# Epiphany-f/PSL-SLAM

Hardware: AMD Instinct MI355X
Metric: frames/sec ORB+line extract+match, 640x480 RGB-D, 1/2/4/8 MI355X (higher is better)
Workload: dtype u8; 1 GPU; configs[2]: 640x480 synthetic structure scene at the configured line load ('sticks': non-overlapping high-contrast bars), ORB 1000/1.2/8 FAST 20/7 + LSD (LSD_REFINE_ADV) / merge / top-200 / LBD + LIL pairing + RGB-D line glue (isLineGood, crossings, planes) extract, SearchByProjection(cur,last) + LSDmatcher::match, frames resident in HBM; scene=sticks, distinct_frames_per_batch=256, streams=1, launcher=none, multi_gpu=single GPU, lsd_refine=LSD_REFINE_ADV, lbd_sample_bytes_per_frame=2654242

## Files before the change

include/pslfe.h:

```cpp
#ifndef PSLFE_H
#define PSLFE_H
#include <stddef.h>
#include <stdint.h>

#ifdef __cplusplus
extern "C" {
#endif

#define PSLFE_OK 0
#define PSLFE_E_INVALID (-1)
#define PSLFE_E_NODEVICE (-2)
#define PSLFE_E_HIP (-3)
#define PSLFE_E_CAPACITY (-4)
#define PSLFE_E_STATE (-5)

#define PSLFE_MAX_LEVELS 16
#define PSLFE_FAN_CAP 4096

typedef struct PslKeyPoint {
    float x, y;
    float size;
    float angle;
    float response;
    int32_t octave;
// ... 78 lines not shown
int pslfe_line_levels(const pslfe_line* line);
float pslfe_line_scale_factor(const pslfe_line* line);
int pslfe_line_scale_factors(const pslfe_line* line, float* scale, float* inv_scale, float* sigma2, float* inv_sigma2);

int pslfe_lsd_detect(pslfe_line* line, const uint8_t* gray, int w, int h, int stride, float* segments, int cap, int* n);
int pslfe_line_debug_gradient(pslfe_line* line, int frame, int* W, int* H, double* scaled, float* angle_deg, double* modgrad);
#define PSLFE_MATH_ATANF 0
#define PSLFE_MATH_TANF 1
#define PSLFE_MATH_SINCOSF 2
#define PSLFE_MATH_FAST_ATAN2 3
#define PSLFE_MATH_ATAN2F 4
#define PSLFE_MATH_FDIV 5
#define PSLFE_MATH_SQRTF 6
#define PSLFE_MATH_CVROUND_F 7
#define PSLFE_MATH_LOG 8
#define PSLFE_MATH_EXP 9
#define PSLFE_MATH_LOG10 10
#define PSLFE_MATH_POW_POS 11
#define PSLFE_MATH_SINH_SMALL 12
#define PSLFE_MATH_LOG_GAMMA 13
#define PSLFE_MATH_GLIBC_SIN 14
#define PSLFE_MATH_GLIBC_COS 15
#define PSLFE_MATH_COS_SIN_F64 16
#define PSLFE_MATH_COS_SIN_2PI_F32 17
#define PSLFE_MATH_RATIO_INV 18
#define PSLFE_MATH_DDIV 19
#define PSLFE_MATH_DSQRT 20
#define PSLFE_MATH_CVROUND_D 21
#define PSLFE_MATH_COUNT 22
int pslfe_debug_math(pslfe_ctx* ctx, int fn, size_t n, const void* a, const void* b, void* out0, void* out1);
#define PSLFE_NFA_FIRST (-2)
int pslfe_line_debug_nfa(pslfe_line* line, int w, int h, int phase, int nframes, const int32_t* nrect, int rect_cap,
                         const double* p_lognfa, const int32_t* nk, double* vals, double* tail, double* log_nt);

int pslfe_line_extract(pslfe_line* line, const uint8_t* gray, int w, int h, int stride, PslKeyLine* kls, uint8_t* desc,
                       double* lineEq, int cap, int* n);
int pslfe_line_extract_batch_device(pslfe_line* line, const uint8_t* d_gray, int nframes, int w, int h, int stride,
                                    size_t frame_stride);
int pslfe_line_results_device(pslfe_line* line, const PslKeyLine** d_kls, const uint8_t** d_desc, const double** d_lineEq,
                              const int32_t** d_counts, int* kl_cap);
int pslfe_line_fetch(pslfe_line* line, int frame, PslKeyLine* kls, uint8_t* desc, double* lineEq, int cap, int* n, int* status);
int pslfe_line_segments_fetch(pslfe_line* line, int frame, float* segments, int cap, int* n);

int pslfe_line_optimize_and_merge(pslfe_line* line, const float* segments, int nseg, int w, int h, PslKeyLine* kls, int cap, int* n);
int pslfe_lbd_compute(pslfe_line* line, const uint8_t* gray, int w, int h, int stride, const PslKeyLine* kls, int nkl,
                      uint8_t* desc, float* fdesc);
int pslfe_line_debug_sobel(pslfe_line* line, int frame, int16_t* dx, int16_t* dy);

int pslfe_lil_pair(pslfe_line* line, const float* lines, int nlines, float radius, float fanThr, int imgCols, int imgRows,
                   float* fans, int cap, int* nfans);
int pslfe_line_pair_batch_device(pslfe_line* line, float radius, float fanThr);
int pslfe_line_fans_fetch(pslfe_line* line, int frame, float* fans, int cap, int* nfans);
int pslfe_line_fans_device(pslfe_line* line, const float** d_fans, const int32_t** d_nfans, int* fan_stride);

int pslfe_line_match_batch_device(pslfe_line* line, int shift, float nnr, int32_t* d_matches12, int32_t* d_nmatches);

int pslfe_hamming_knn2(pslfe_ctx* ctx, const uint8_t* q, int nq, const uint8_t* t, int nt,
                       int32_t* idx, int32_t* dist);
int pslfe_hamming_knn2_device(pslfe_ctx* ctx, const uint8_t* d_q, int nq, const uint8_t* d_t, int nt,
                              int32_t* d_idx, int32_t* d_dist);

typedef struct PslProjQuery {
    float u, v;
    float radius;
    float ur;
    int32_t min_level;
// ... 559 lines not shown
```

psl-slam_amd/__init__.py:

```python
import ctypes as C
import os

import numpy as np

_HERE = os.path.dirname(os.path.abspath(__file__))
LIB_PATH = os.path.join(_HERE, "libpslfe.so")

KEYPOINT_DTYPE = np.dtype([("x", "<f4"), ("y", "<f4"), ("size", "<f4"), ("angle", "<f4"), ("response", "<f4"),
                           ("octave", "<i4"), ("class_id", "<i4")])
KEYLINE_DTYPE = np.dtype([("angle", "<f4"), ("class_id", "<i4"), ("octave", "<i4"), ("pt_x", "<f4"), ("pt_y", "<f4"),
                          ("response", "<f4"), ("size", "<f4"), ("startPointX", "<f4"), ("startPointY", "<f4"),
                          ("endPointX", "<f4"), ("endPointY", "<f4"), ("sPointInOctaveX", "<f4"),
                          ("sPointInOctaveY", "<f4"), ("ePointInOctaveX", "<f4"), ("ePointInOctaveY", "<f4"),
                          ("lineLength", "<f4"), ("numOfPixels", "<i4")])
PROJQUERY_DTYPE = np.dtype([("u", "<f4"), ("v", "<f4"), ("radius", "<f4"), ("ur", "<f4"), ("min_level", "<i4"),
                            ("max_level", "<i4"), ("angle", "<f4"), ("blocks", "<i4")])
BOWQUERY_DTYPE = np.dtype([("start", "<i4"), ("len", "<i4"), ("angle", "<f4")])
CAMERA_DTYPE = np.dtype([(k, "<f4") for k in ("fx", "fy", "cx", "cy", "k1", "k2", "p1", "p2", "k3", "bf")])
assert KEYPOINT_DTYPE.itemsize == 28 and KEYLINE_DTYPE.itemsize == 68 and PROJQUERY_DTYPE.itemsize == 32
POSE_DTYPE = np.dtype([("R", "<f4", (9,)), ("t", "<f4", (3,))])
LASTPOINT_DTYPE = np.dtype([("x", "<f4"), ("y", "<f4"), ("z", "<f4"), ("state", "<i4")])
MAPPOINT_DTYPE = np.dtype([(k, "<f4") for k in ("x", "y", "z", "nx", "ny", "nz", "min_dist", "max_dist")])
assert POSE_DTYPE.itemsize == 48 and LASTPOINT_DTYPE.itemsize == 16 and MAPPOINT_DTYPE.itemsize == 32
LASTPOINT_NONE, LASTPOINT_NO_OBS, LASTPOINT_OBS, LASTPOINT_OUTLIER = 0, 1, 2, 8
# ... 1250 lines not shown
    else:
        assert b is None, f"{fn} takes one argument"
    return MATH_FUNCTIONS.index(fn), a, b, np.zeros(len(a), t0), None if t1 is None else np.zeros(len(a), t1)


def debug_math(fn, a, b=None, ctx=None):
    ctx = ctx or default_context()
    i, a, b, o0, o1 = math_arrays(fn, a, b)
    _check(lib().pslfe_debug_math(ctx._h, C.c_int(i), C.c_size_t(len(a)), _ptr(a), _ptr(b), _ptr(o0), _ptr(o1)), "pslfe_debug_math")
    return o0 if o1 is None else (o0, o1)


NFA_FIRST = -2


def _line_debug_nfa(self, w, h, phase, nrect, p_lognfa, nk):
    nrect = np.ascontiguousarray(nrect, np.int32).ravel()
    F = len(nrect)
    pl = np.ascontiguousarray(p_lognfa, np.float64)
    nk = np.ascontiguousarray(nk, np.int32)
    R = pl.shape[1]
    assert pl.shape == (F, R, 2) and nk.shape == (F, R, 5, 2), (pl.shape, nk.shape)
    vals = np.full((F, R, 5), np.nan)
    tail = np.full((F, R, 5), np.nan)
    lognt = C.c_double()
    _check(lib().pslfe_line_debug_nfa(self._h, C.c_int(w), C.c_int(h), C.c_int(phase), C.c_int(F), _ptr(nrect), C.c_int(R), _ptr(pl), _ptr(nk),
                                      _ptr(vals), _ptr(tail), C.byref(lognt)), "pslfe_line_debug_nfa")
    return vals, tail, lognt.value


LINEextractor.debug_nfa = _line_debug_nfa


def _lsd_search_by_geom_appearance(self, kl_last, desc_last, kl_cur, desc_cur, has_mapline, desc_th, bounds):
    k1 = np.ascontiguousarray(kl_last, KEYLINE_DTYPE)
    k2 = np.ascontiguousarray(kl_cur, KEYLINE_DTYPE)
    d1 = np.ascontiguousarray(desc_last, np.uint8).reshape(-1, 32)
    d2 = np.ascontiguousarray(desc_cur, np.uint8).reshape(-1, 32)
    hm = np.ascontiguousarray(has_mapline, np.uint8)
    m12 = np.full(max(len(k1), 1), -1, np.int32)
    asg = np.full(max(len(k2), 1), -1, np.int32)
    n = C.c_int()
    _check(lib().pslfe_line_search_by_geom_appearance(self.ctx._h, _ptr(k1), _ptr(d1), C.c_int(len(k1)), _ptr(k2), _ptr(d2), C.c_int(len(k2)),
                                                      _ptr(hm), C.c_float(desc_th), *[C.c_float(b) for b in bounds], _ptr(m12), _ptr(asg),
                                                      C.byref(n)), "pslfe_line_search_by_geom_appearance")
    return n.value, m12[:len(k1)], asg[:len(k2)]


def _lsd_frame_bf_match(self, ldesc1, ldesc2, TH):
    d1 = np.ascontiguousarray(ldesc1, np.uint8).reshape(-1, 32)
    d2 = np.ascontiguousarray(ldesc2, np.uint8).reshape(-1, 32)
    lm = np.full(max(len(d1), 1), -1, np.int32)
    _check(lib().pslfe_line_frame_bf_match(self.ctx._h, _ptr(d1), C.c_int(len(d1)), _ptr(d2), C.c_int(len(d2)), C.c_float(self.mfNNratio),
                                           C.c_float(TH), _ptr(lm)), "pslfe_line_frame_bf_match")
    return lm[:len(d1)]


LSDmatcher.SearchByGeomNApearance = _lsd_search_by_geom_appearance
LSDmatcher.FrameBFMatch = _lsd_frame_bf_match


def associate_planes(planes, points, map_planes, dTh, aTh, live=True, map_bad=None, ctx=None):
    ctx = ctx or default_context()
    p = np.ascontiguousarray(planes, np.float32).reshape(-1, 4)
    q = np.ascontiguousarray(points, np.float64).reshape(-1, 15)
    m = np.ascontiguousarray(map_planes, np.float32).reshape(-1, 4)
# ... 748 lines not shown
```

psl-slam_amd/csrc/line_kernels3.h:

```cpp
#ifndef PSL_LINE_KERNELS3_H
#define PSL_LINE_KERNELS3_H

#include "line_kernels.h"
#include "psl_log_gamma.h"

struct LsdnRect { double x1, y1, x2, y2, width, theta, dx, dy, prec, p; };
struct LsdnGeom {
    int ya, yb;
    int lefty, righty;
    long long minx, fl, sl, fr, sr;
};

__device__ __forceinline__ void lsdn_cswap(long long& a, long long& b) { const long long lo = a < b ? a : b, hi = a < b ? b : a; a = lo; b = hi; }

__device__ __forceinline__ void lsdn_geom(const LsdnRect& r, int H, LsdnGeom* G) {
    const double half_width = r.width / 2.0;
    const double dyhw = PSL_DMUL(r.dy, half_width), dxhw = PSL_DMUL(r.dx, half_width);
    int cx[4] = {(int)PSL_DSUB(r.x1, dyhw), (int)PSL_DSUB(r.x2, dyhw), (int)PSL_DADD(r.x2, dyhw), (int)PSL_DADD(r.x1, dyhw)};
    int cy[4] = {(int)PSL_DADD(r.y1, dxhw), (int)PSL_DADD(r.y2, dxhw), (int)PSL_DSUB(r.y2, dxhw), (int)PSL_DSUB(r.y1, dxhw)};
    long long k[4];
#pragma unroll
    for (int i = 0; i < 4; ++i) k[i] = (long long)cx[i] * 4294967296ll + ((long long)cy[i] + 2147483648ll);
    lsdn_cswap(k[0], k[1]); lsdn_cswap(k[2], k[3]); lsdn_cswap(k[0], k[2]); lsdn_cswap(k[1], k[3]); lsdn_cswap(k[1], k[2]);
#pragma unroll
// ... 33 lines not shown
    G->yb = mxy >= H ? H - 1 : mxy;
}

__device__ __forceinline__ void lsdn_row_span(const LsdnGeom& G, int y, int W, int* xa, int* xb) {
    const int n = y - G.ya;
    int c1 = (y < G.lefty ? y : G.lefty) - G.ya; c1 = c1 < 0 ? 0 : c1;
    int d1 = (y < G.righty ? y : G.righty) - G.ya; d1 = d1 < 0 ? 0 : d1;
    const long long L = G.minx + G.fl * c1 + G.sl * (n - c1);
    const long long R = G.minx + G.fr * d1 + G.sr * (n - d1);
    *xa = (int)(L < 0 ? 0 : (L > W ? W : L));
    *xb = (int)(R >= W ? W - 1 : (R < -1 ? -1 : R));
}

#ifndef PSL_NFA_BYROW_MIN
#define PSL_NFA_BYROW_MIN 4
#endif
#ifndef PSL_NFA_BYROW_T
#define PSL_NFA_BYROW_T 3
#endif
template <int GL>
__device__ __forceinline__ int lsdn_group_sum(int v) {
#pragma unroll
    for (int o = GL / 2; o > 0; o >>= 1) v += __shfl_xor(v, o);
    return v;
}

template <int GL>
__device__ __forceinline__ int lsdn_group_max(int v) {
#pragma unroll
    for (int o = GL / 2; o > 0; o >>= 1) { const int u = __shfl_xor(v, o); v = u > v ? u : v; }
    return v;
}

template <int NP, int GL>
__device__ __forceinline__ void lsdn_count(const float* __restrict__ ang, int W, const LsdnGeom& G, double theta, const double* prec, int lane, int* total, int* alg) {
    int al[NP];
#pragma unroll
    for (int j = 0; j < NP; ++j) al[j] = 0;
    const float theta_deg = (float)(theta * 57.295779513082320877);
    float pdeg[NP];
#pragma unroll
    for (int j = 0; j < NP; ++j) pdeg[j] = (float)(prec[j] * 57.295779513082320877);
    auto pixel = [&](float a) {
        if (a == PSL_LSD_NOTDEF) return;
        float d = __builtin_fabsf(theta_deg - a);
        const float d2 = __builtin_fabsf(d - 360.0f);
        d = d > 270.0f ? d2 : d;
        bool close = __builtin_fabsf(d - 270.0f) < 2e-3f;
#pragma unroll
        for (int j = 0; j < NP; ++j) close = close || __builtin_fabsf(d - pdeg[j]) < 2e-3f;
        if (!close) {
#pragma unroll
            for (int j = 0; j < NP; ++j) al[j] += d <= pdeg[j] ? 1 : 0;
        } else {
            const double f = lsdg_fold(PSL_DMUL((double)a, PSL_DEG2RAD), theta);
#pragma unroll
            for (int j = 0; j < NP; ++j) al[j] += f <= prec[j] ? 1 : 0;
        }
    };
    const int nrows = G.yb - G.ya + 1;
    int tot = 0;
    if (nrows >= PSL_NFA_BYROW_MIN) {
        for (int y = G.ya + lane; y <= G.yb; y += GL) {
            int xa, xb;
            lsdn_row_span(G, y, W, &xa, &xb);
            const int c = xb - xa + 1;
            tot += c > 0 ? c : 0;
            const float* row = ang + y * W;
            for (int x = xa; x <= xb; x += 4) {
                float a[4];
#pragma unroll
                for (int u = 0; u < 4; ++u) a[u] = x + u <= xb ? row[x + u] : PSL_LSD_NOTDEF;
#pragma unroll
                for (int u = 0; u < 4; ++u) pixel(a[u]);
            }
        }
        *total = lsdn_group_sum<GL>(tot);
    } else {
        int wmax = 0;
        for (int y = G.ya + lane; y <= G.yb; y += GL) {
            int xa, xb;
            lsdn_row_span(G, y, W, &xa, &xb);
            const int c = xb - xa + 1;
            tot += c > 0 ? c : 0;
            wmax = c > wmax ? c : wmax;
        }
        *total = lsdn_group_sum<GL>(tot);
        wmax = lsdn_group_max<GL>(wmax);
        if (nrows > 0 && wmax > 0) {
            const int nslots = nrows * wmax, row_step = GL / wmax, dx_step = GL - row_step * wmax;
            int row = lane / wmax, dx = lane - row * wmax;
            for (int s = lane; s < nslots; s += 4 * GL) {
                float a[4];
#pragma unroll
                for (int u = 0; u < 4; ++u) {
                    a[u] = PSL_LSD_NOTDEF;
                    if (s + GL * u < nslots) {
                        int xa, xb;
                        const int y = G.ya + row;
                        lsdn_row_span(G, y, W, &xa, &xb);
                        if (dx <= xb - xa) a[u] = ang[y * W + xa + dx];
                    }
                    dx += dx_step; row += row_step;
                    if (dx >= wmax) { dx -= wmax; ++row; }
                }
#pragma unroll
                for (int u = 0; u < 4; ++u) pixel(a[u]);
            }
        }
    }
#pragma unroll
    for (int j = 0; j < NP; ++j) alg[j] = lsdn_group_sum<GL>(al[j]);
}

struct LsdnGeomI { int ya, yb, lefty, righty, minx, fl, sl, fr, sr; };
typedef __attribute__((address_space(3))) const int lds_cint;

__device__ __forceinline__ void lsdn_row_span_i(lds_cint* g, int y, int W, int* xa, int* xb) {
    const int ya = g[0], lefty = g[2], righty = g[3], minx = g[4];
    const int n = y - ya;
    int c1 = (y < lefty ? y : lefty) - ya; c1 = c1 < 0 ? 0 : c1;
    int d1 = (y < righty ? y : righty) - ya; d1 = d1 < 0 ? 0 : d1;
    const int L = minx + g[5] * c1 + g[6] * (n - c1);
    const int R = minx + g[7] * d1 + g[8] * (n - d1);
    *xa = L < 0 ? 0 : (L > W ? W : L);
    *xb = R >= W ? W - 1 : (R < -1 ? -1 : R);
}

template <int GL>
__device__ __forceinline__ void lsdn_count_trials(const float* __restrict__ ang, int W, lds_cint* geo, double theta, double prec, int lane, int* total, int* alg) {
    const float theta_deg = (float)(theta * 57.295779513082320877), pdeg = (float)(prec * 57.295779513082320877);
    auto aligned = [&](float a) -> bool {
        if (a == PSL_LSD_NOTDEF) return false;
        float d = __builtin_fabsf(theta_deg - a);
        const float d2 = __builtin_fabsf(d - 360.0f);
        d = d > 270.0f ? d2 : d;
        if (__builtin_fabsf(d - 270.0f) < 2e-3f || __builtin_fabsf(d - pdeg) < 2e-3f) return lsdg_fold(PSL_DMUL((double)a, PSL_DEG2RAD), theta) <= prec;
        return d <= pdeg;
    };
    int ya = 0, yb = -1;
    bool any = false;
#pragma unroll
    for (int t = 0; t < 5; ++t) {
        const int a = geo[9 * t], b = geo[9 * t + 1];
        if (b >= a) {
            ya = !any || a < ya ? a : ya;
            yb = !any || b > yb ? b : yb;
            any = true;
        }
    }
    int tot[5], al[5];
#pragma unroll
    for (int t = 0; t < 5; ++t) { tot[t] = 0; al[t] = 0; }
    const bool by_row = yb - ya + 1 >= PSL_NFA_BYROW_T;
    for (int y = by_row ? ya + lane : ya; y <= yb; y += by_row ? GL : 1) {
        int xa[5], xb[5], ua = 0x7fffffff, ub = -1;
#pragma unroll
        for (int t = 0; t < 5; ++t) {
            xa[t] = 1; xb[t] = 0;
            if (y >= geo[9 * t] && y <= geo[9 * t + 1]) lsdn_row_span_i(geo + 9 * t, y, W, &xa[t], &xb[t]);
            if (xb[t] >= xa[t]) {
                if (by_row || lane == 0) tot[t] += xb[t] - xa[t] + 1;
                ua = xa[t] < ua ? xa[t] : ua; ub = xb[t] > ub ? xb[t] : ub;
            }
        }
        if (ub < ua) continue;
        const float* row = ang + y * W;
        const int step = by_row ? 1 : GL;
        for (int x = by_row ? ua : ua + lane; x <= ub; x += 4 * step) {
            float a[4];
#pragma unroll
            for (int u = 0; u < 4; ++u) a[u] = x + step * u <= ub ? row[x + step * u] : PSL_LSD_NOTDEF;
#pragma unroll
            for (int u = 0; u < 4; ++u) {
                if (aligned(a[u])) {
#pragma unroll
                    for (int t = 0; t < 5; ++t) al[t] += (x + step * u >= xa[t] && x + step * u <= xb[t]) ? 1 : 0;
                }
            }
        }
    }
#pragma unroll
    for (int t = 0; t < 5; ++t) { total[t] = lsdn_group_sum<GL>(tot[t]); alg[t] = lsdn_group_sum<GL>(al[t]); }
}

__device__ __forceinline__ bool lsdn_double_equal0(double a) {
    if (a == 0.0) return true;
    const double aa = fabs(a);
    const double abs_max = aa < 2.2250738585072014e-308 ? 2.2250738585072014e-308 : aa;
    return (aa / abs_max) <= PSL_DMUL(100.0, 2.2204460492503131e-16);
}

#define PSL_NFA_NP 11
struct LsdnTables {
    const double* lg;
    const double* logs;
    int lg_n;
    double p0, log_nt;
    const double* inv;
};

__device__ __forceinline__ double lsdn_lg(const LsdnTables& T, int i) { return i < T.lg_n ? T.lg[i] : lsdn_log_gamma((double)i); }

__device__ __forceinline__ int lsdn_tail_test_fast(double term, double bin_tail, double mult_term, int q, double log_nt) {
    const unsigned long long bits = (unsigned long long)__double_as_longlong(bin_tail);
    const int e = (int)((bits >> 52) & 0x7ff) - 1023;
    if (e <= -1022 || e >= 1024 || q < 2) return -1;
    const double tb = 0.1 * bin_tail;
    {
        const double a0 = -(double)e * 0.30102999566398120 - log_nt, a1 = -(double)(e + 1) * 0.30102999566398120 - log_nt;
        const double f0 = fabs(a0), f1 = fabs(a1);
// ... 32 lines not shown
__device__ __forceinline__ void lsdn_load(const double* __restrict__ r, LsdnRect* rec) {
    rec->x1 = r[0]; rec->y1 = r[1]; rec->x2 = r[2]; rec->y2 = r[3]; rec->width = r[4]; rec->theta = r[5]; rec->dx = r[6]; rec->dy = r[7];
    rec->prec = r[8]; rec->p = r[9];
}

#ifndef PSL_NFA_GL
#define PSL_NFA_GL 16
#endif

#ifndef PSL_NFA_COUNT_WAVES
#define PSL_NFA_COUNT_WAVES 8
#endif
template <int PH>
__global__ __launch_bounds__(256, PSL_NFA_COUNT_WAVES) void k_lsd_nfa_count(LineParams P, const float* __restrict__ angdeg, double* __restrict__ rects,
                                                          const int* __restrict__ nrect, const uint16_t* __restrict__ ulist, const int* __restrict__ ucount,
                                                          int2* __restrict__ counts, int2* __restrict__ count0) {
    static_assert(PH == PSL_NFA_FIRST || (PH >= 0 && PH <= 3), "phase -1 is counted by the first test's pass");
    constexpr int GPB = 256 / PSL_NFA_GL;
    __shared__ int s_geo[GPB * 45];
    const int frame = blockIdx.y, lane = threadIdx.x & (PSL_NFA_GL - 1);
    const int cnt = PH == PSL_NFA_FIRST ? (nrect[frame] < P.maxseg ? nrect[frame] : P.maxseg) : ucount[frame];
    const uint16_t* ul = ulist + (size_t)frame * P.maxseg;
    const float* ang = angdeg + (size_t)frame * P.W * P.H;
    for (int item = (int)blockIdx.x * GPB + (int)(threadIdx.x / PSL_NFA_GL); item < cnt; item += (int)gridDim.x * GPB) {
        const int idx = PH == PSL_NFA_FIRST ? item : (int)ul[item];
        const size_t o = (size_t)frame * P.maxseg + idx;
        double* rs = rects + o * PSL_LSD_RECT_F64;
        LsdnRect rec;
        lsdn_load(rs, &rec);
        LsdnGeom G;
        int2* out = counts + o * 5;
        if (PH == PSL_NFA_FIRST) {
            if (lane == 0) { rs[8] = P.prec; rs[9] = P.p; }
            double pr[6], pp = P.p;
            pr[0] = P.prec;
#pragma unroll
            for (int t = 0; t < 5; ++t) { pp = pp / 2; pr[t + 1] = PSL_DMUL(pp, PSL_PI); }
            int tot, kk[6];
            lsdn_geom(rec, P.H, &G);
            lsdn_count<6, PSL_NFA_GL>(ang, P.W, G, rec.theta, pr, lane, &tot, kk);
            if (lane == 0) {
                count0[o] = make_int2(tot, kk[0]);
#pragma unroll
                for (int t = 0; t < 5; ++t) out[t] = make_int2(tot, kk[t + 1]);
            }
        } else if (PH == 3) {
            if (!(PSL_DSUB(rec.width, 0.5) >= 0.5)) {
                if (lane < 5) out[lane] = make_int2(-1, 0);
                continue;
            }
            double pr[5], pp = rec.p;
#pragma unroll
            for (int t = 0; t < 5; ++t) { pp = pp / 2; pr[t] = PSL_DMUL(pp, PSL_PI); }
            int tot, kk[5];
            lsdn_geom(rec, P.H, &G);
            lsdn_count<5, PSL_NFA_GL>(ang, P.W, G, rec.theta, pr, lane, &tot, kk);
            if (lane == 0) {
#pragma unroll
                for (int t = 0; t < 5; ++t) out[t] = make_int2(tot, kk[t]);
            }
        } else {
            int* geo = &s_geo[(threadIdx.x / PSL_NFA_GL) * 45];
            if (lane < 5) {
                LsdnRect r = rec;
                bool valid = true;
                for (int t = 0; t <= lane; ++t) {
                    if (!(PSL_DSUB(r.width, 0.5) >= 0.5)) { valid = false; break; }
                    lsdn_shrink(r, PH);
                }
                int* g = geo + 9 * lane;
                g[0] = 0; g[1] = -2;
                if (valid) {
                    lsdn_geom(r, P.H, &G);
                    g[1] = -1;
                    if (G.yb >= G.ya) {
                        g[0] = G.ya; g[1] = G.yb; g[2] = G.lefty; g[3] = G.righty; g[4] = (int)G.minx;
                        g[5] = (int)G.fl; g[6] = (int)G.sl; g[7] = (int)G.fr; g[8] = (int)G.sr;
                    }
                }
            }
            __builtin_amdgcn_wave_barrier();
            int nn[5], kk[5];
            lsdn_count_trials<PSL_NFA_GL>(ang, P.W, (lds_cint*)geo, rec.theta, rec.prec, lane, nn, kk);
            if (lane == 0) {
#pragma unroll
                for (int t = 0; t < 5; ++t) out[t] = geo[9 * t + 1] == -2 ? make_int2(-1, 0) : make_int2(nn[t], kk[t]);
            }
            __builtin_amdgcn_wave_barrier();
        }
// ... 289 lines not shown
```

psl-slam_amd/csrc/pslfe_line.hip:

```cpp
#include <math.h>
#include <stdlib.h>
#include <string.h>

#include <algorithm>
#include <mutex>
#include <vector>

#include "line_kernels2.h"
#include "line_kernels3.h"
#include "pslfe_internal.h"

#ifndef PSL_NFA_COUNT_WGS
#define PSL_NFA_COUNT_WGS 4
#endif
#define PSL_GROW_LDS_USED_MAX (144u * 1024u)
#ifndef PSL_GROW_HELPER_FRAMES
#define PSL_GROW_HELPER_FRAMES 64
#endif
constexpr unsigned PSL_LINE_PIECES = 2;
constexpr unsigned PSL_LINE_FIRST_NUM = 7, PSL_LINE_FIRST_DEN = 12;

#define PSL_GROW_LDS_DEVICES 64
static std::mutex g_grow_lds_mu;
static size_t g_grow_lds_attr[PSL_GROW_LDS_DEVICES];
// ... 65 lines not shown
    float* d_tmplines = nullptr;

    PslDeviceBuffers mem;

    void release() {
        mem.release();
        gw = gh = 0;
        last_nframes = 0;
    }

    int prepare(int w, int h) {
        if (w == gw && h == gh) return PSLFE_OK;
        PSL_REQUIRE(w >= 16 && h >= 16 && w <= 8192 && h <= 8192, PSLFE_E_INVALID, "line: image %dx%d out of range", w, h);
        LineParams Q;
        memset(&Q, 0, sizeof(Q));
        Q.w = w; Q.h = h;
        Q.W = (int)nearbyint(w * 0.8);
        Q.H = (int)nearbyint(h * 0.8);
        Q.maxseg = PSL_MERGE_NMAX;
        Q.maxkl = std::max(1024, nfeatures);
        Q.nfeatures = nfeatures;
        {
            const double sigma = 0.6 / 0.8;
            const int ksize = 1 + 2 * (int)ceil(sigma * sqrt(2 * 3.0 * log(10.0)));
            PSL_REQUIRE(ksize == 7, PSLFE_E_INVALID, "line: unexpected LSD kernel size %d", ksize);
            const double scale2X = -0.5 / (sigma * sigma);
            double sum = 0;
            for (int i = 0; i < 7; ++i) { const double x = i - 3.0; Q.gk[i] = exp(scale2X * x * x); sum += Q.gk[i]; }
            sum = 1. / sum;
            for (int i = 0; i < 7; ++i) Q.gk[i] *= sum;
        }
        Q.prec = PSL_PI * 22.5 / 180;
        Q.p = 22.5 / 180;
        Q.rho = 2.0 / sin(Q.prec);
        {
            double q = Q.rho * Q.rho;
            while (sqrt(nextafter(q, INFINITY)) <= Q.rho) q = nextafter(q, INFINITY);
            while (sqrt(q) > Q.rho) q = nextafter(q, 0.0);
            Q.rho_q = q;
        }
        const double LOG_NT = 5 * (log10((double)Q.W) + log10((double)Q.H)) / 2 + log10(11.0);
        Q.min_reg_size = (int)(size_t)(-LOG_NT / log10(Q.p));
        Q.log_nt = LOG_NT;
        Q.refine = refine;
        {
            float cf[5];
            double sum = 0;
            for (int i = 0; i < 5; ++i) { const double x = i - 2.0; cf[i] = (float)exp(-0.5 * x * x); sum += cf[i]; }
            sum = 1. / sum;
            for (int i = 0; i < 5; ++i) { cf[i] = (float)(cf[i] * sum); Q.lbdK[i] = (int)nearbyint((double)cf[i] * 256.0); }
        }
        {
            const int wb = 7, nb = 9;
            double u = (wb * 3 - 1) / 2, sigma = (wb * 2 + 1) / 2, inv = -1 / (2 * sigma * sigma);
            for (int i = 0; i < wb * 3; ++i) { const double d = i - u; Q.gaussL[i] = (float)exp(d * d * inv); }
            u = (nb * wb - 1) / 2; sigma = u; inv = -1 / (2 * sigma * sigma);
            for (int i = 0; i < nb * wb; ++i) { const double d = i - u; Q.gaussG[i] = (float)exp(d * d * inv); }
        }
        PSL_HIP(hipSetDevice(ctx->device));
        PSL_HIP(hipStreamSynchronize(ctx->stream));
        release();
        if (int rc = allocate(Q, w, h)) { release(); return rc; }
        P = Q;
        gw = w; gh = h;
        last_nframes = 0;
        return PSLFE_OK;
// ... 454 lines not shown
    }
#define PSL_NFA_DEBUG_EVAL(PH)                                                                                                                  \
    case PH:                                                                                                                                    \
        k_lsd_nfa_setup<PH><<<F, 256, 0, st>>>(P, line->NT, line->d_rects, line->d_nrect, d_ul, d_uc, line->d_counts, line->d_count0, line->d_vals, \
                                               line->d_sstate, line->d_stmp, line->d_slist, line->d_lcount);                                    \
        k_lsd_nfa_series<PH><<<dim3(PSL_NFA_NCLS, (F + PSL_NFA_FG - 1) / PSL_NFA_FG), 256, 0, st>>>(P, line->NT, (int)F, line->d_slist, line->d_lcount, \
                                                                                                    line->d_sstate);                            \
        break;
    switch (phase) {
        PSL_NFA_DEBUG_EVAL(PSL_NFA_FIRST)
        PSL_NFA_DEBUG_EVAL(-1)
        PSL_NFA_DEBUG_EVAL(0)
        PSL_NFA_DEBUG_EVAL(1)
        PSL_NFA_DEBUG_EVAL(2)
        PSL_NFA_DEBUG_EVAL(3)
    }
#undef PSL_NFA_DEBUG_EVAL
    PSL_HIP(hipGetLastError());
    std::vector<double> v(F * N * 5);
    std::vector<double2> ss(F * N * 5);
    PSL_HIP(hipMemcpyAsync(v.data(), line->d_vals, v.size() * sizeof(double), hipMemcpyDeviceToHost, st));
    PSL_HIP(hipMemcpyAsync(ss.data(), line->d_sstate, ss.size() * sizeof(double2), hipMemcpyDeviceToHost, st));
    PSL_HIP(hipStreamSynchronize(st));
    for (size_t f = 0; f < F; ++f)
        for (int r = 0; r < nrect[f]; ++r)
            for (int t = 0; t < TR; ++t) {
                vals[((size_t)f * rect_cap + r) * 5 + t] = v[(f * N + r) * 5 + t];
                tail[((size_t)f * rect_cap + r) * 5 + t] = ss[(f * N + r) * 5 + t].x;
            }
    if (log_nt) *log_nt = line->NT.log_nt;
    return PSLFE_OK;
}

int pslfe_line_extract_batch_device(pslfe_line* line, const uint8_t* d_gray, int nframes, int w, int h, int stride, size_t frame_stride) {
    PSL_REQUIRE(line && d_gray, PSLFE_E_INVALID, "pslfe_line_extract_batch_device: NULL argument");
    PSL_REQUIRE(nframes >= 1 && nframes <= line->max_batch, PSLFE_E_INVALID, "pslfe_line_extract_batch_device: nframes %d (max_batch %d)", nframes, line->max_batch);
    PSL_REQUIRE(stride >= w && (nframes == 1 || frame_stride >= (size_t)stride * h), PSLFE_E_INVALID, "pslfe_line_extract_batch_device: strides");
    return line->run_extract(d_gray, nframes, w, h, stride, frame_stride);
}

int pslfe_line_results_device(pslfe_line* line, const PslKeyLine** d_kls, const uint8_t** d_desc, const double** d_lineEq,
                              const int32_t** d_counts, int* kl_cap) {
    PSL_REQUIRE(line, PSLFE_E_INVALID, "pslfe_line_results_device: line is NULL");
    PSL_REQUIRE(line->last_nframes > 0, PSLFE_E_STATE, "pslfe_line_results_device: no batch extracted yet");
    if (d_kls) *d_kls = line->d_kls;
    if (d_desc) *d_desc = line->d_ldesc;
    if (d_lineEq) *d_lineEq = line->d_lineEq;
    if (d_counts) *d_counts = line->d_nkl;
    if (kl_cap) *kl_cap = line->P.maxkl;
    return PSLFE_OK;
}

int pslfe_line_fetch(pslfe_line* line, int frame, PslKeyLine* kls, uint8_t* desc, double* lineEq, int cap, int* n, int* status) {
    PSL_REQUIRE(line && n, PSLFE_E_INVALID, "pslfe_line_fetch: NULL argument");
    PSL_REQUIRE(line->last_nframes > 0 && frame >= 0 && frame < line->last_nframes, PSLFE_E_STATE, "pslfe_line_fetch: frame %d", frame);
    PSL_HIP(hipSetDevice(line->ctx->device));
    hipStream_t st = line->ctx->stream;
    int cnt = 0, stt = 0;
    PSL_HIP(hipMemcpyAsync(&cnt, line->d_nkl + frame, sizeof(int), hipMemcpyDeviceToHost, st));
    PSL_HIP(hipMemcpyAsync(&stt, line->d_status + frame, sizeof(int), hipMemcpyDeviceToHost, st));
    PSL_HIP(hipStreamSynchronize(st));
    *n = cnt;
    if (status) *status = stt;
    PSL_REQUIRE(cnt <= cap, PSLFE_E_CAPACITY, "pslfe_line_fetch: %d keylines, capacity %d", cnt, cap);
    if (cnt > 0) {
        const size_t o = (size_t)frame * line->P.maxkl;
// ... 179 lines not shown
```

Before: 36860 frames/s.

## Bin NFA alignment counts via exponent-bit histogram and bitmask popcounts

The LSD NFA count kernel used to compare each pixel's angle difference against every halved tolerance. Because those tolerances are successive powers of two, it now computes the bin straight from the float exponent bits and accumulates into a packed 64-bit histogram of 10-bit fields, flushed before any field can overflow. A double-precision fallback handles values near a bin edge. The refine counter builds a 32-bit aligned-pixel mask and uses popcount against span bitmasks in place of per-pixel comparisons over five ranges. A debug entry point and a startup check on the factor-of-two tolerance relation are also added.

```diff
diff --git a/include/pslfe.h b/include/pslfe.h
--- a/include/pslfe.h
+++ b/include/pslfe.h
@@ -134,6 +134,8 @@
 #define PSLFE_NFA_FIRST (-2)
 int pslfe_line_debug_nfa(pslfe_line* line, int w, int h, int phase, int nframes, const int32_t* nrect, int rect_cap,
                          const double* p_lognfa, const int32_t* nk, double* vals, double* tail, double* log_nt);
+int pslfe_line_debug_nfa_count(pslfe_line* line, int w, int h, int phase, int nframes, const int32_t* nrect, int rect_cap,
+                               const double* rects, const float* angle_deg, int32_t* nk, int32_t* first_nk);
 
 int pslfe_line_extract(pslfe_line* line, const uint8_t* gray, int w, int h, int stride, PslKeyLine* kls, uint8_t* desc,
                        double* lineEq, int cap, int* n);
diff --git a/psl-slam_amd/__init__.py b/psl-slam_amd/__init__.py
--- a/psl-slam_amd/__init__.py
+++ b/psl-slam_amd/__init__.py
@@ -1306,6 +1306,24 @@
 LINEextractor.debug_nfa = _line_debug_nfa
 
 
+def _line_debug_nfa_count(self, w, h, phase, nrect, rects, angle_deg):
+    nrect = np.ascontiguousarray(nrect, np.int32).ravel()
+    F = len(nrect)
+    rects = np.ascontiguousarray(rects, np.float64)
+    ang = np.ascontiguousarray(angle_deg, np.float32)
+    R = rects.shape[1]
+    W, H = int(round(w * 0.8)), int(round(h * 0.8))
+    assert rects.shape == (F, R, 12) and ang.shape == (F, H, W), (rects.shape, ang.shape, (F, H, W))
+    nk = np.full((F, R, 5, 2), -2, np.int32)
+    first = np.full((F, R, 2), -2, np.int32) if phase == NFA_FIRST else None
+    _check(lib().pslfe_line_debug_nfa_count(self._h, C.c_int(w), C.c_int(h), C.c_int(phase), C.c_int(F), _ptr(nrect), C.c_int(R), _ptr(rects),
+                                            _ptr(ang), _ptr(nk), _ptr(first) if first is not None else None), "pslfe_line_debug_nfa_count")
+    return nk, first
+
+
+LINEextractor.debug_nfa_count = _line_debug_nfa_count
+
+
 def _lsd_search_by_geom_appearance(self, kl_last, desc_last, kl_cur, desc_cur, has_mapline, desc_th, bounds):
     k1 = np.ascontiguousarray(kl_last, KEYLINE_DTYPE)
     k2 = np.ascontiguousarray(kl_cur, KEYLINE_DTYPE)
diff --git a/psl-slam_amd/csrc/line_kernels3.h b/psl-slam_amd/csrc/line_kernels3.h
--- a/psl-slam_amd/csrc/line_kernels3.h
+++ b/psl-slam_amd/csrc/line_kernels3.h
@@ -89,47 +89,67 @@
     return v;
 }
 
-template <int NP, int GL>
-__device__ __forceinline__ void lsdn_count(const float* __restrict__ ang, int W, const LsdnGeom& G, double theta, const double* prec, int lane, int* total, int* alg) {
-    int al[NP];
-#pragma unroll
-    for (int j = 0; j < NP; ++j) al[j] = 0;
+#define LSDN_FW 10
+#define LSDN_CAP ((1 << LSDN_FW) - 1)
+#define LSDN_SEG 1020
+static_assert(LSDN_SEG <= LSDN_CAP && LSDN_SEG % 4 == 0, "a piece of a row must fit in a histogram field");
+template <int NP, bool FIRST, int GL>
+__device__ __forceinline__ void lsdn_count(const float* __restrict__ ang, int W, const LsdnGeom& G, double theta, double prec0, double p, int lane, int* total, int* alg) {
+    static_assert(NP * LSDN_FW <= 64, "the histogram is one 64-bit register pair");
+    int cnt[NP];
+#pragma unroll
+    for (int f = 0; f < NP; ++f) cnt[f] = 0;
+    unsigned long long hist = 0;
+    auto flush = [&]() {
+#pragma unroll
+        for (int f = 0; f < NP; ++f) cnt[f] += (int)((hist >> (LSDN_FW * f)) & LSDN_CAP);
+        hist = 0;
+    };
     const float theta_deg = (float)(theta * 57.295779513082320877);
-    float pdeg[NP];
-#pragma unroll
-    for (int j = 0; j < NP; ++j) pdeg[j] = (float)(prec[j] * 57.295779513082320877);
+    constexpr int NH = FIRST ? NP - 1 : NP;
+    const double half = PSL_DMUL(p / 2, PSL_PI);
+    const float top = (float)((FIRST ? prec0 : half) * 57.295779513082320877);
+    const int topbits = __float_as_int(top);
+    const float margin = top >= 8e-3f * (float)(1 << NP) ? 2e-3f : __builtin_inff();
     auto pixel = [&](float a) {
         if (a == PSL_LSD_NOTDEF) return;
         float d = __builtin_fabsf(theta_deg - a);
         const float d2 = __builtin_fabsf(d - 360.0f);
         d = d > 270.0f ? d2 : d;
-        bool close = __builtin_fabsf(d - 270.0f) < 2e-3f;
-#pragma unroll
-        for (int j = 0; j < NP; ++j) close = close || __builtin_fabsf(d - pdeg[j]) < 2e-3f;
-        if (!close) {
-#pragma unroll
-            for (int j = 0; j < NP; ++j) al[j] += d <= pdeg[j] ? 1 : 0;
-        } else {
+        int c = ((topbits - __float_as_int(d)) >> 23) + 1;
+        c = c < 0 ? 0 : (c > NP ? NP : c);
+        const int lobits = topbits - (c << 23);
+        const float lo = __int_as_float(lobits), hi = __int_as_float(lobits + (1 << 23));
+        const float near = __builtin_fminf(__builtin_fminf(__builtin_fabsf(d - lo), __builtin_fabsf(d - hi)), __builtin_fabsf(d - 270.0f));
+        if (near < margin) {
             const double f = lsdg_fold(PSL_DMUL((double)a, PSL_DEG2RAD), theta);
-#pragma unroll
-            for (int j = 0; j < NP; ++j) al[j] += f <= prec[j] ? 1 : 0;
-        }
+            const long long e = ((__double_as_longlong(half) - __double_as_longlong(f)) >> 52) + 1;
+            c = e < 0 ? 0 : (e > NH ? NH : (int)e);
+            if (FIRST) c += f <= prec0 ? 1 : 0;
+        }
+        hist += 1ull << (LSDN_FW * NP - LSDN_FW * c);
     };
     const int nrows = G.yb - G.ya + 1;
     int tot = 0;
     if (nrows >= PSL_NFA_BYROW_MIN) {
+        int pend = 0;
         for (int y = G.ya + lane; y <= G.yb; y += GL) {
             int xa, xb;
             lsdn_row_span(G, y, W, &xa, &xb);
             const int c = xb - xa + 1;
             tot += c > 0 ? c : 0;
             const float* row = ang + y * W;
-            for (int x = xa; x <= xb; x += 4) {
-                float a[4];
-#pragma unroll
-                for (int u = 0; u < 4; ++u) a[u] = x + u <= xb ? row[x + u] : PSL_LSD_NOTDEF;
-#pragma unroll
-                for (int u = 0; u < 4; ++u) pixel(a[u]);
+            for (int x0 = xa; x0 <= xb; x0 += LSDN_SEG) {
+                const int xe = xb - x0 >= LSDN_SEG ? x0 + LSDN_SEG - 1 : xb;
+                if (pend + (xe - x0 + 1) > LSDN_CAP) { flush(); pend = 0; }
+                pend += xe - x0 + 1;
+                for (int x = x0; x <= xe; x += 4) {
+                    float a[4];
+#pragma unroll
+                    for (int u = 0; u < 4; ++u) a[u] = x + u <= xe ? row[x + u] : PSL_LSD_NOTDEF;
+#pragma unroll
+                    for (int u = 0; u < 4; ++u) pixel(a[u]);
+                }
             }
         }
         *total = lsdn_group_sum<GL>(tot);
@@ -147,27 +167,35 @@
         if (nrows > 0 && wmax > 0) {
             const int nslots = nrows * wmax, row_step = GL / wmax, dx_step = GL - row_step * wmax;
             int row = lane / wmax, dx = lane - row * wmax;
-            for (int s = lane; s < nslots; s += 4 * GL) {
-                float a[4];
-#pragma unroll
-                for (int u = 0; u < 4; ++u) {
-                    a[u] = PSL_LSD_NOTDEF;
-                    if (s + GL * u < nslots) {
-                        int xa, xb;
-                        const int y = G.ya + row;
-                        lsdn_row_span(G, y, W, &xa, &xb);
-                        if (dx <= xb - xa) a[u] = ang[y * W + xa + dx];
+            for (int s0 = lane; s0 < nslots; s0 += LSDN_SEG * GL) {
+                const int se = nslots - s0 > LSDN_SEG * GL ? s0 + LSDN_SEG * GL : nslots;
+                for (int s = s0; s < se; s += 4 * GL) {
+                    float a[4];
+#pragma unroll
+                    for (int u = 0; u < 4; ++u) {
+                        a[u] = PSL_LSD_NOTDEF;
+                        if (s + GL * u < nslots) {
+                            int xa, xb;
+                            const int y = G.ya + row;
+                            lsdn_row_span(G, y, W, &xa, &xb);
+                            if (dx <= xb - xa) a[u] = ang[y * W + xa + dx];
+                        }
+                        dx += dx_step; row += row_step;
+                        if (dx >= wmax) { dx -= wmax; ++row; }
                     }
-                    dx += dx_step; row += row_step;
-                    if (dx >= wmax) { dx -= wmax; ++row; }
-                }
-#pragma unroll
-                for (int u = 0; u < 4; ++u) pixel(a[u]);
-            }
-        }
-    }
-#pragma unroll
-    for (int j = 0; j < NP; ++j) alg[j] = lsdn_group_sum<GL>(al[j]);
+#pragma unroll
+                    for (int u = 0; u < 4; ++u) pixel(a[u]);
+                }
+                flush();
+            }
+        }
+    }
+    flush();
+#pragma unroll
+    for (int f = 0; f < NP; ++f) cnt[f] = lsdn_group_sum<GL>(cnt[f]);
+    int run = 0;
+#pragma unroll
+    for (int j = NP - 1; j >= 0; --j) { run += cnt[NP - 1 - j]; alg[j] = run; }
 }
 
 struct LsdnGeomI { int ya, yb, lefty, righty, minx, fl, sl, fr, sr; };
@@ -182,6 +210,12 @@
     const int R = minx + g[7] * d1 + g[8] * (n - d1);
     *xa = L < 0 ? 0 : (L > W ? W : L);
     *xb = R >= W ? W - 1 : (R < -1 ? -1 : R);
+}
+
+__device__ __forceinline__ unsigned lsdn_span_bits(int lo, int hi) {
+    lo = lo < 0 ? 0 : lo;
+    hi = hi > 31 ? 31 : hi;
+    return hi >= lo ? (0xffffffffu >> (31 - hi + lo)) << lo : 0u;
 }
 
 template <int GL>
@@ -223,17 +257,24 @@
         }
         if (ub < ua) continue;
         const float* row = ang + y * W;
-        const int step = by_row ? 1 : GL;
-        for (int x = by_row ? ua : ua + lane; x <= ub; x += 4 * step) {
-            float a[4];
-#pragma unroll
-            for (int u = 0; u < 4; ++u) a[u] = x + step * u <= ub ? row[x + step * u] : PSL_LSD_NOTDEF;
-#pragma unroll
-            for (int u = 0; u < 4; ++u) {
-                if (aligned(a[u])) {
-#pragma unroll
-                    for (int t = 0; t < 5; ++t) al[t] += (x + step * u >= xa[t] && x + step * u <= xb[t]) ? 1 : 0;
-                }
+        const int step = by_row ? 1 : GL, sh = by_row ? 0 : __builtin_ctz(GL);
+        for (int x0 = by_row ? ua : ua + lane; x0 <= ub; x0 += 32 * step) {
+            unsigned m = 0;
+#pragma unroll 1
+            for (int i = 0; i < 32 && x0 + step * i <= ub; i += 4) {
+                const int x = x0 + step * i;
+                float a[4];
+#pragma unroll
+                for (int u = 0; u < 4; ++u) a[u] = x + step * u <= ub ? row[x + step * u] : PSL_LSD_NOTDEF;
+#pragma unroll
+                for (int u = 0; u < 4; ++u) {
+                    if (aligned(a[u])) m |= 1u << (i + u);
+                }
+            }
+            if (m != 0) {
+#pragma unroll
+                for (int t = 0; t < 5; ++t)
+                    al[t] += __builtin_popcount(m & lsdn_span_bits((xa[t] - x0 + step - 1) >> sh, (xb[t] - x0) >> sh));
             }
         }
     }
@@ -332,13 +373,9 @@
         int2* out = counts + o * 5;
         if (PH == PSL_NFA_FIRST) {
             if (lane == 0) { rs[8] = P.prec; rs[9] = P.p; }
-            double pr[6], pp = P.p;
-            pr[0] = P.prec;
-#pragma unroll
-            for (int t = 0; t < 5; ++t) { pp = pp / 2; pr[t + 1] = PSL_DMUL(pp, PSL_PI); }
             int tot, kk[6];
             lsdn_geom(rec, P.H, &G);
-            lsdn_count<6, PSL_NFA_GL>(ang, P.W, G, rec.theta, pr, lane, &tot, kk);
+            lsdn_count<6, true, PSL_NFA_GL>(ang, P.W, G, rec.theta, P.prec, P.p, lane, &tot, kk);
             if (lane == 0) {
                 count0[o] = make_int2(tot, kk[0]);
 #pragma unroll
@@ -349,12 +386,9 @@
                 if (lane < 5) out[lane] = make_int2(-1, 0);
                 continue;
             }
-            double pr[5], pp = rec.p;
-#pragma unroll
-            for (int t = 0; t < 5; ++t) { pp = pp / 2; pr[t] = PSL_DMUL(pp, PSL_PI); }
             int tot, kk[5];
             lsdn_geom(rec, P.H, &G);
-            lsdn_count<5, PSL_NFA_GL>(ang, P.W, G, rec.theta, pr, lane, &tot, kk);
+            lsdn_count<5, false, PSL_NFA_GL>(ang, P.W, G, rec.theta, 0.0, rec.p, lane, &tot, kk);
             if (lane == 0) {
 #pragma unroll
                 for (int t = 0; t < 5; ++t) out[t] = make_int2(tot, kk[t]);
diff --git a/psl-slam_amd/csrc/pslfe_line.hip b/psl-slam_amd/csrc/pslfe_line.hip
--- a/psl-slam_amd/csrc/pslfe_line.hip
+++ b/psl-slam_amd/csrc/pslfe_line.hip
@@ -121,6 +121,8 @@
         }
         Q.prec = PSL_PI * 22.5 / 180;
         Q.p = 22.5 / 180;
+        PSL_REQUIRE((float)(Q.prec * 57.295779513082320877) == 2.0f * (float)((Q.p / 2 * PSL_PI) * 57.295779513082320877), PSLFE_E_INVALID,
+                    "line: the first test's tolerance is not twice phase -1's first one in f32 degrees");
         Q.rho = 2.0 / sin(Q.prec);
         {
             double q = Q.rho * Q.rho;
@@ -641,6 +643,79 @@
     return PSLFE_OK;
 }
 
+int pslfe_line_debug_nfa_count(pslfe_line* line, int w, int h, int phase, int nframes, const int32_t* nrect, int rect_cap, const double* rects,
+                               const float* angle_deg, int32_t* nk, int32_t* first_nk) {
+    PSL_REQUIRE(line && nrect && rects && angle_deg && nk, PSLFE_E_INVALID, "pslfe_line_debug_nfa_count: NULL argument");
+    PSL_REQUIRE(phase == PSL_NFA_FIRST || (phase >= 0 && phase <= 3), PSLFE_E_INVALID, "pslfe_line_debug_nfa_count: phase %d (phase -1 is counted by the first test's pass)", phase);
+    PSL_REQUIRE(phase != PSL_NFA_FIRST || first_nk, PSLFE_E_INVALID, "pslfe_line_debug_nfa_count: the first test needs first_nk");
+    PSL_REQUIRE(nframes >= 1 && nframes <= line->max_batch, PSLFE_E_INVALID, "pslfe_line_debug_nfa_count: nframes %d (max_batch %d)", nframes, line->max_batch);
+    PSL_REQUIRE(rect_cap >= 1 && rect_cap <= PSL_MERGE_NMAX, PSLFE_E_INVALID, "pslfe_line_debug_nfa_count: rect_cap %d (at most %d)", rect_cap, PSL_MERGE_NMAX);
+    for (int f = 0; f < nframes; ++f)
+        PSL_REQUIRE(nrect[f] >= 0 && nrect[f] <= rect_cap, PSLFE_E_INVALID, "pslfe_line_debug_nfa_count: frame %d has %d rectangles (rect_cap %d)", f, nrect[f], rect_cap);
+    for (int f = 0; f < nframes; ++f)
+        for (int r = 0; r < nrect[f]; ++r) {
+            const double* q = rects + ((size_t)f * rect_cap + r) * PSL_LSD_RECT_F64;
+            bool ok = true;
+            for (int i = 0; i < 10; ++i) ok = ok && std::isfinite(q[i]);
+            for (int i = 0; i < 5; ++i) ok = ok && fabs(q[i]) <= 32768.0;
+            ok = ok && fabs(q[6]) <= 1.0 && fabs(q[7]) <= 1.0 && q[8] > 0.0 && q[9] > 0.0 && q[9] < 1.0;
+            PSL_REQUIRE(ok, PSLFE_E_INVALID, "pslfe_line_debug_nfa_count: frame %d rectangle %d is not a rectangle of the grower's kind", f, r);
+        }
+    int rc = line->prepare(w, h);
+    if (rc) return rc;
+    PSL_HIP(hipSetDevice(line->ctx->device));
+    hipStream_t st = line->ctx->stream;
+    const LineParams& P = line->P;
+    const size_t F = (size_t)nframes, N = (size_t)P.maxseg, npx = (size_t)P.W * P.H;
+    std::vector<double> rs(F * N * PSL_LSD_RECT_F64, 0.0);
+    std::vector<uint16_t> ulist(F * N, 0);
+    for (size_t f = 0; f < F; ++f)
+        for (int r = 0; r < nrect[f]; ++r) {
+            memcpy(&rs[(f * N + r) * PSL_LSD_RECT_F64], rects + (f * rect_cap + r) * PSL_LSD_RECT_F64, PSL_LSD_RECT_F64 * sizeof(double));
+            ulist[f * N + r] = (uint16_t)(nrect[f] - 1 - r);
+        }
+    PSL_HIP(hipMemcpyAsync(line->d_rects, rs.data(), rs.size() * sizeof(double), hipMemcpyHostToDevice, st));
+    PSL_HIP(hipMemcpyAsync(line->d_nrect, nrect, F * sizeof(int), hipMemcpyHostToDevice, st));
+    PSL_HIP(hipMemcpyAsync(line->d_angdeg, angle_deg, F * npx * sizeof(float), hipMemcpyHostToDevice, st));
+    PSL_HIP(hipMemsetAsync(line->d_counts, 0xff, F * N * 5 * sizeof(int2), st));
+    uint16_t* d_ul = nullptr;
+    int* d_uc = nullptr;
+    if (phase != PSL_NFA_FIRST) {
+        d_ul = line->d_ulist + (size_t)((phase + 1) & 1) * N * F;
+        d_uc = line->d_ucount + (size_t)(phase + 1) * F;
+        PSL_HIP(hipMemcpyAsync(d_ul, ulist.data(), ulist.size() * sizeof(uint16_t), hipMemcpyHostToDevice, st));
+        PSL_HIP(hipMemcpyAsync(d_uc, nrect, F * sizeof(int), hipMemcpyHostToDevice, st));
+    }
+    const dim3 gc(F >= 64 ? PSL_NFA_COUNT_WGS : 128, (unsigned)F);
+#define PSL_NFA_DEBUG_COUNT(PH)                                                                                                       \
+    case PH:                                                                                                                          \
+        k_lsd_nfa_count<PH><<<gc, 256, 0, st>>>(P, line->d_angdeg, line->d_rects, line->d_nrect, d_ul, d_uc, line->d_counts, line->d_count0); \
+        break;
+    switch (phase) {
+        PSL_NFA_DEBUG_COUNT(PSL_NFA_FIRST)
+        PSL_NFA_DEBUG_COUNT(0)
+        PSL_NFA_DEBUG_COUNT(1)
+        PSL_NFA_DEBUG_COUNT(2)
+        PSL_NFA_DEBUG_COUNT(3)
+    }
+#undef PSL_NFA_DEBUG_COUNT
+    PSL_HIP(hipGetLastError());
+    std::vector<int2> c(F * N * 5), c0(phase == PSL_NFA_FIRST ? F * N : 0);
+    PSL_HIP(hipMemcpyAsync(c.data(), line->d_counts, c.size() * sizeof(int2), hipMemcpyDeviceToHost, st));
+    if (!c0.empty()) PSL_HIP(hipMemcpyAsync(c0.data(), line->d_count0, c0.size() * sizeof(int2), hipMemcpyDeviceToHost, st));
+    PSL_HIP(hipStreamSynchronize(st));
+    line->last_nframes = 0;
+    for (size_t f = 0; f < F; ++f)
+        for (int r = 0; r < nrect[f]; ++r) {
+            for (int t = 0; t < 5; ++t) {
+                nk[((f * rect_cap + r) * 5 + t) * 2] = c[(f * N + r) * 5 + t].x;
+                nk[((f * rect_cap + r) * 5 + t) * 2 + 1] = c[(f * N + r) * 5 + t].y;
+            }
+            if (!c0.empty()) { first_nk[(f * rect_cap + r) * 2] = c0[f * N + r].x; first_nk[(f * rect_cap + r) * 2 + 1] = c0[f * N + r].y; }
+        }
+    return PSLFE_OK;
+}
+
 int pslfe_line_extract_batch_device(pslfe_line* line, const uint8_t* d_gray, int nframes, int w, int h, int stride, size_t frame_stride) {
     PSL_REQUIRE(line && d_gray, PSLFE_E_INVALID, "pslfe_line_extract_batch_device: NULL argument");
     PSL_REQUIRE(nframes >= 1 && nframes <= line->max_batch, PSLFE_E_INVALID, "pslfe_line_extract_batch_device: nframes %d (max_batch %d)", nframes, line->max_batch);
```

Result: no change. 37160 frames/s (median of 6 runs) (+0.8%).
